# chellmuth/pathed

Hardware: AMD Instinct MI355X
Metric: Msamples/s (pixels x spp / s), PathTracer radiance loop (higher is better)
Workload: dtype f32; 1 GPU; scenes/cornell.json 1024x1024, 1024 spp per step x 8 steps = 8192 spp, bounces 0..10, seed 1; total_samples=8589934592, parallelism=the samples of every step split over 1 GPU(s), no exchange

## Files before the change

### include/pathed_hip.h

```cpp
#ifndef PATHED_HIP_H
#define PATHED_HIP_H

#include <stddef.h>
#include <stdint.h>

#ifdef __cplusplus
extern "C" {
#endif

#define PATHED_ABI_VERSION 4

#define PATHED_OK            0
#define PATHED_E_INVALID    -1
#define PATHED_E_DEVICE     -2
#define PATHED_E_NO_DEVICE  -3
#define PATHED_E_UNSUPPORTED -4
#define PATHED_E_NOMEM      -5

#define PATHED_MAT_LAMBERTIAN 0
#define PATHED_MAT_OREN_NAYAR 1
#define PATHED_MAT_MICROFACET 2
#define PATHED_MAT_PLASTIC    3
#define PATHED_MAT_GLASS      4
#define PATHED_MAT_MIRROR     5
// ... 270 lines not shown
};
enum {
    PATHED_TRAITS_ALL = 0, PATHED_TRAITS_LAMBERTIAN_TRIANGLES = 1, PATHED_TRAITS_LAMBERTIAN_PLASTIC_SPHERES = 2,
    PATHED_TRAITS_LAMBERTIAN_GLASS_CONTAINER = 3, PATHED_TRAITS_TRIANGLE_LIT = 4, PATHED_TRAITS_ENVIRONMENT_ONLY = 5,
    PATHED_TRAITS_ROUGH_BECKMANN = 6, PATHED_TRAITS_ROUGH_GGX = 7, PATHED_TRAITS_SMOOTH = 8, PATHED_TRAITS_COUNT = 9
};
int pathed_hip_debug_shading_queries(PathedScene *scene, int function, int traits, size_t n, const float *in, float *out);

int pathed_hip_debug_phase_samples(PathedScene *scene, size_t n, const float *u, float *out);

int pathed_hip_trace(PathedScene *scene, const float *rays, size_t n,
                     int any_hit, void *hits);

int pathed_hip_debug_small_candidates(PathedScene *scene, const float *rays, size_t n, uint64_t *out);

int pathed_hip_debug_camera_masks(PathedScene *scene, uint64_t *out, size_t n_pixels);

int pathed_hip_debug_item_order(PathedScene *scene, int32_t *primitives, size_t n_triangles);

int pathed_hip_debug_light_records(PathedScene *scene, float *triangles, size_t n_triangles, float *lights, size_t max_lights, int *n_lights);

int pathed_hip_debug_instance_records(PathedScene *scene, float *records , size_t n_instances);

int pathed_hip_has_experiments(void);

int pathed_hip_set_stats_mode(PathedScene *scene, int enabled);
int pathed_hip_get_stats(PathedScene *scene, PathedStats *out);
int pathed_hip_reset_stats(PathedScene *scene);

int pathed_hip_scene_export_bvh(PathedScene *scene,
// ... 40 lines not shown
```

### pathed_amd/_capi.py

```python
import ctypes as C
import os

_HERE = os.path.dirname(os.path.abspath(__file__))
REPO_ROOT = os.path.dirname(_HERE)
LIB_DIR = os.path.join(_HERE, "lib")

PATHED_ABI_VERSION = 4

MAT_LAMBERTIAN, MAT_OREN_NAYAR, MAT_MICROFACET, MAT_PLASTIC, MAT_GLASS, MAT_MIRROR, MAT_PASSTHROUGH = range(7)
INTEGRATOR_PATH_TRACER, INTEGRATOR_VOLUME_PATH_TRACER, INTEGRATOR_ALBEDO, INTEGRATOR_BASIC_VOLUME = 0, 1, 2, 3
ALBEDO_CONSTANT, ALBEDO_CHECKERBOARD, ALBEDO_TEXTURE = 0, 1, 2
GEOM_MESH, GEOM_SPHERE = 0, 1


class PathedCamera(C.Structure):
    _fields_ = [
        ("origin", C.c_float * 3),
        ("target", C.c_float * 3),
        ("up", C.c_float * 3),
        ("vertical_fov", C.c_float),
        ("width", C.c_int32),
        ("height", C.c_int32),
        ("flip_handedness", C.c_int32),
    ]
# ... 211 lines not shown
    "pathed_hip_grid_queries",
    "pathed_hip_debug_shading_queries",
    "pathed_hip_debug_phase_samples",
    "pathed_hip_scene_destroy",
    "pathed_hip_render",
    "pathed_hip_render_device",
    "pathed_hip_render_features",
    "pathed_hip_render_features_device",
    "pathed_hip_render_moments",
    "pathed_hip_render_moments_device",
    "pathed_hip_noise_estimate_device",
    "pathed_hip_select_pixels_device",
    "pathed_hip_render_pixels_device",
    "pathed_hip_trace",
    "pathed_hip_debug_small_candidates",
    "pathed_hip_debug_camera_masks",
    "pathed_hip_debug_item_order",
    "pathed_hip_debug_light_records",
    "pathed_hip_has_experiments",
    "pathed_hip_scene_refit",
    "pathed_hip_set_samples_per_unit",
    "pathed_hip_set_integrator",
    "pathed_hip_set_stats_mode",
    "pathed_hip_get_stats",
    "pathed_hip_reset_stats",
    "pathed_hip_scene_export_bvh",
    "pathed_hip_scene_export_compressed_nodes",
    "pathed_hip_measure_bandwidth",
    "pathed_hip_measure_valu",
    "pathed_hip_measure_valu_modes",
# ... 102 lines not shown
        lib.pathed_hip_render_moments_device.argtypes = [vp, C.c_uint64, C.c_uint32, C.c_uint32, C.c_int, C.c_int, vp, vp, vp]
        lib.pathed_hip_render_moments_device.restype = C.c_int
        lib.pathed_hip_render_moments.argtypes = [vp, C.c_uint64, C.c_uint32, C.c_uint32, C.c_int, C.c_int, fp, fp]
        lib.pathed_hip_render_moments.restype = C.c_int
        lib.pathed_hip_noise_estimate_device.argtypes = [vp, vp, vp, C.c_uint32, C.c_float, C.c_float, vp, C.POINTER(PathedNoise), vp]
        lib.pathed_hip_noise_estimate_device.restype = C.c_int
    if hasattr(lib, "pathed_hip_render_pixels_device"):
        lib.pathed_hip_select_pixels_device.argtypes = [vp, vp, vp, vp, C.c_float, C.c_float, vp, vp, C.POINTER(C.c_uint32), C.POINTER(PathedNoise), vp]
        lib.pathed_hip_select_pixels_device.restype = C.c_int
        lib.pathed_hip_render_pixels_device.argtypes = [vp, C.c_uint64, C.c_uint32, C.c_uint32, C.c_int, C.c_int, vp, C.c_uint32, vp, vp, vp, vp]
        lib.pathed_hip_render_pixels_device.restype = C.c_int
    lib.pathed_hip_trace.argtypes = [vp, C.POINTER(C.c_float), C.c_size_t, C.c_int, vp]
    lib.pathed_hip_trace.restype = C.c_int
    lib.pathed_hip_debug_small_candidates.argtypes = [vp, C.POINTER(C.c_float), C.c_size_t, C.POINTER(C.c_uint64)]
    lib.pathed_hip_debug_small_candidates.restype = C.c_int
    lib.pathed_hip_debug_light_records.argtypes = [vp, C.POINTER(C.c_float), C.c_size_t, C.POINTER(C.c_float), C.c_size_t, C.POINTER(C.c_int)]
    lib.pathed_hip_debug_light_records.restype = C.c_int
    if hasattr(lib, "pathed_hip_debug_camera_masks"):
        lib.pathed_hip_debug_camera_masks.argtypes = [vp, C.POINTER(C.c_uint64), C.c_size_t]
        lib.pathed_hip_debug_camera_masks.restype = C.c_int
        lib.pathed_hip_debug_item_order.argtypes = [vp, C.POINTER(C.c_int32), C.c_size_t]
        lib.pathed_hip_debug_item_order.restype = C.c_int
    if hasattr(lib, "pathed_hip_debug_shading_queries"):
        lib.pathed_hip_debug_shading_queries.argtypes = [vp, C.c_int, C.c_int, C.c_size_t, C.POINTER(C.c_float), C.POINTER(C.c_float)]
        lib.pathed_hip_debug_shading_queries.restype = C.c_int
    if hasattr(lib, "pathed_hip_debug_phase_samples"):
        lib.pathed_hip_debug_phase_samples.argtypes = [vp, C.c_size_t, C.POINTER(C.c_float), C.POINTER(C.c_float)]
        lib.pathed_hip_debug_phase_samples.restype = C.c_int
    lib.pathed_hip_scene_refit.argtypes = [vp, C.POINTER(C.c_float), C.POINTER(C.c_float), C.c_uint32, C.POINTER(C.c_float)]
    lib.pathed_hip_scene_refit.restype = C.c_int
# ... 79 lines not shown
```

### pathed_amd/csrc/kernels.h

```cpp
#pragma once

#ifndef PATHED_RESOLVE_SHARED
#define PATHED_RESOLVE_SHARED 2
#endif
#ifndef PATHED_EXPERIMENTS
#define PATHED_EXPERIMENTS 0
#endif
#include "mfma_candidates.h"
#include "small_items.h"
#include "camera_masks.h"
#include "shading.h"
#include "trace.h"
#include "volume.h"

namespace pathed {

static const int kBlock = 256;
static_assert(kBlock == kVolumeBlock, "volume.h indexes the LDS stack rows with the block size");
static const int kWavesPerBlock = kBlock / 64;
static const int kMaxLdsMaterials = 96;
#ifndef PATHED_UNIT_QUEUES
#define PATHED_UNIT_QUEUES 32
#endif
static const int kUnitQueues = PATHED_UNIT_QUEUES;
// ... 733 lines not shown
    } else {
        aHigh = 0u;
        bHigh = 0u;
    }
    *lowA = aLow; *highA = aHigh; *lowB = bLow; *highB = bHigh;
}

__device__ __forceinline__ unsigned int shiftInBit(unsigned int word, unsigned long long laneMask)
{
    unsigned int result;
    unsigned long long carryOut;
    asm("v_addc_co_u32_e64 %0, %1, %2, %2, %3" : "=v"(result), "=s"(carryOut) : "v"(word), "s"(laneMask));
    return result;
}

template <bool SHADOW, bool QUADS = true, bool LONE = true>
__device__ __forceinline__ void smallCandidatesItems(const f2 *records, int nQuads, int nTris, float kappaT, V3 origin, V3 directionA, V3 directionB,
                                                     unsigned int *lowA, unsigned int *highA, unsigned int *lowB, unsigned int *highB,
                                                     float tnearLow, float tfarHighB)
{
    unsigned int loA = 0u, hiA = 0u, loB = 0u, hiB = 0u;
    const f2 ax = splat2(directionA.x), ay = splat2(directionA.y), az = splat2(directionA.z);
    const f2 bx = splat2(directionB.x), by = splat2(directionB.y), bz = splat2(directionB.z);
    const f2 ox = splat2(origin.x), oy = splat2(origin.y), oz = splat2(origin.z);
    const f2 nearLow = splat2(-tnearLow), farHighB = splat2(fminf(tfarHighB, 1e30f));
    const f2 kappaLength = splat2(kappaT);

    const int nQuadPairs = QUADS ? (nQuads + 1) >> 1 : 0;
    for (int pair = 0; QUADS && pair < nQuadPairs; pair++) {
        const f2 *record = records + kSmallQuadWords * pair;
        const f2 c0x = record[0], c0y = record[1], c0z = record[2];
        const f2 a1x = record[3], a1y = record[4], a1z = record[5];
        const f2 a2x = record[6], a2y = record[7], a2z = record[8];
        const f2 k2UV = record[9], amaxSquared = record[10], k2T = record[11], cD = record[13], kappaUV = record[15];
        const f2 tx = ox - c0x, ty = oy - c0y, tz = oz - c0z;
        const f2 qx = fma2(ty, a1z, -(tz * a1y));
        const f2 qy = fma2(tz, a1x, -(tx * a1z));
        const f2 qz = fma2(tx, a1y, -(ty * a1x));
        const f2 tScaled = fma2(a2x, qx, fma2(a2y, qy, a2z * qz));
        const f2 tt = fma2(tx, tx, fma2(ty, ty, tz * tz));
        const f2 reachSquared = tt + amaxSquared;
        const f2 originUV = k2UV * reachSquared, originT = k2T * reachSquared;
        auto oneRay = [&](f2 dx, f2 dy, f2 dz, bool far, unsigned int &lo, unsigned int &hi) {
            const f2 px = fma2(dy, a2z, -(dz * a2y));
// ... 17 lines not shown
                const f2 farBound = fma2(farHighB, det, -tScaled) * det;
                const f2 tolFar = fma2(farHighB, fma2(splat2(kSmallKappaFar), dd, cD), tolT);
                rejectX |= PATHED_LANES(farBound.x < -tolFar.x);
                rejectY |= PATHED_LANES(farBound.y < -tolFar.y);
            }
            const f2 twice = tolUV + tolUV;
            const float twiceX = twice.x, twiceY = twice.y;
            hi = __builtin_amdgcn_alignbit(hi, lo, 28);
            lo = shiftInBit(lo, ~(rejectX | PATHED_LANES(diagonal.x < -twiceX)));
            lo = shiftInBit(lo, ~(rejectX | PATHED_LANES(diagonal.x > twiceX)));
            lo = shiftInBit(lo, ~(rejectY | PATHED_LANES(diagonal.y < -twiceY)));
            lo = shiftInBit(lo, ~(rejectY | PATHED_LANES(diagonal.y > twiceY)));
        };
        oneRay(ax, ay, az, false, loA, hiA);
        __builtin_amdgcn_sched_barrier(0);
        if (SHADOW) { oneRay(bx, by, bz, true, loB, hiB); }
        __builtin_amdgcn_sched_barrier(0);
    }
    unsigned long long accA, accB;
    if (QUADS && (nQuads & 1)) {
        accA = (((unsigned long long)hiA << 32) | loA) >> 2; accB = (((unsigned long long)hiB << 32) | loB) >> 2;
        loA = (unsigned int)accA; hiA = (unsigned int)(accA >> 32); loB = (unsigned int)accB; hiB = (unsigned int)(accB >> 32);
    }

    const f2 *lone = records + kSmallQuadWords * nQuadPairs;
    const int nLone = LONE ? nTris - 2 * nQuads : 0;
    const int nLonePairs = (nLone + 1) >> 1;
    for (int pair = 0; LONE && pair < nLonePairs; pair++) {
        const f2 *record = lone + kSmallPairWords * pair;
        const f2 v0x = record[0], v0y = record[1], v0z = record[2];
        const f2 e1x = record[3], e1y = record[4], e1z = record[5];
        const f2 e2x = record[6], e2y = record[7], e2z = record[8];
        const f2 tx = ox - v0x, ty = oy - v0y, tz = oz - v0z;
        const f2 qx = fma2(ty, e1z, -(tz * e1y));
// ... 9 lines not shown
            const f2 vScaled = fma2(dx, qx, fma2(dy, qy, dz * qz));
            const f2 a = uScaled * det, b = vScaled * det, c = (det - (uScaled + vScaled)) * det, e = fma2(nearLow, det, tScaled) * det;
            float worstA = fminf(fminf(a.x, b.x), fminf(c.x, e.x));
            float worstB = fminf(fminf(a.y, b.y), fminf(c.y, e.y));
            if (far) {
                const f2 g = fma2(splat2(tfarHighB), det, -tScaled) * det;
                worstA = fminf(worstA, g.x);
                worstB = fminf(worstB, g.y);
            }
            hi = __builtin_amdgcn_alignbit(hi, lo, 30);
            lo = shiftInBit(lo, ~PATHED_LANES(worstA < 0.f));
            lo = shiftInBit(lo, ~PATHED_LANES(worstB < 0.f));
            #undef PATHED_LANES
        };
        oneRay(ax, ay, az, false, loA, hiA);
        if (SHADOW) { oneRay(bx, by, bz, true, loB, hiB); }
    }
    accA = ((unsigned long long)hiA << 32) | loA; accB = ((unsigned long long)hiB << 32) | loB;
    if (LONE && (nLone & 1)) { accA >>= 1; accB >>= 1; }

    const int shift = 64 - nTris;
    accA <<= shift;
    accB <<= shift;
    *lowA = (unsigned int)(accA >> 32); *highA = (unsigned int)accA; *lowB = (unsigned int)(accB >> 32); *highB = (unsigned int)accB;
}

__device__ __forceinline__ void smallResolve(const TraceGeometry &geometry, LaneRay &ray, unsigned int candidatesLow, unsigned int candidatesHigh)
{
    while (__ballot((candidatesLow | candidatesHigh) != 0u) != 0ull) {
        if ((candidatesLow | candidatesHigh) != 0u) {
            int k;
            if (candidatesLow != 0u) { k = __clz((int)candidatesLow); candidatesLow &= ~(0x80000000u >> k); }
            else { k = __clz((int)candidatesHigh); candidatesHigh &= ~(0x80000000u >> k); k += 32; }
            const float4 t0 = geometry.tris[3 * k + 0];
            const float4 t1 = geometry.tris[3 * k + 1];
            const float4 t2 = geometry.tris[3 * k + 2];
            bool terminate = false;
            testLeafTriangle(ray, t0, t1, t2, &terminate);
            if (terminate) { candidatesLow = 0u; candidatesHigh = 0u; }
        }
// ... 1974 lines not shown
        LaneRay ray;
        laneRayInit(ray, path.o, path.d, PATHED_TNEAR, PATHED_TFAR, false);
        {
            const bool traceShadow = tracing && pendingShadow;
            LaneRay shadowRay;
            laneRayInit(shadowRay, path.o, shadowDirection, PATHED_TNEAR, shadowTfar, true);
            unsigned int candidatesLow = 0, candidatesHigh = 0, shadowLow = 0, shadowHigh = 0;
            SHADE_REGION(2, traceShadow);
            if (MFMA) {
                mfmaCandidatesPair(mfmaRows, nTris, p.mfmaFrame, __ballot(traceShadow) != 0ull, path.o, path.d, shadowDirection,
                                   candidateNear(PATHED_TNEAR), candidateFar(shadowTfar), &candidatesLow, &candidatesHigh, &shadowLow, &shadowHigh);
                if (!tracing) { candidatesLow = 0u; candidatesHigh = 0u; }
                if (!traceShadow) { shadowLow = 0u; shadowHigh = 0u; }
            } else if (QUADS) {
                if (tracing) {
                    smallCandidatesItems<true, true, true>(smallTris.data, p.smallQuads, nTris, p.smallKappaT, path.o, path.d, shadowDirection,
                                                            &candidatesLow, &candidatesHigh, &shadowLow, &shadowHigh,
                                                            candidateNear(PATHED_TNEAR), candidateFar(shadowTfar));
                    if (!traceShadow) { shadowLow = 0u; shadowHigh = 0u; }
                }
            } else if (__ballot(traceShadow) != 0ull) {
                if (tracing) {
                    smallCandidatesPair(smallTris.data, nTris, path.o, path.d, shadowDirection, &candidatesLow, &candidatesHigh, &shadowLow, &shadowHigh,
                                        candidateNear(PATHED_TNEAR), candidateFar(shadowTfar));
                    if (!traceShadow) { shadowLow = 0u; shadowHigh = 0u; }
                }
            } else if (tracing) {
                smallCandidates(smallTris.data, nTris, path.o, path.d, &candidatesLow, &candidatesHigh, candidateNear(PATHED_TNEAR));
            }
            if (COUNT && tracing) {
                trisTested += (unsigned int)nTris * (traceShadow ? 2u : 1u);
                closestRays++;
                if (traceShadow) { shadowRays++; }
// ... 158 lines not shown
        if (((k < 32 ? aLow : aHigh) >> (31 - (k & 31))) & 1u) { valuA |= bit; }
        if (((k < 32 ? bLow : bHigh) >> (31 - (k & 31))) & 1u) { valuB |= bit; }
        if ((((k & 1) ? oddA : evenA) >> (k >> 1)) & 1u) { mfmaA |= bit; }
        if ((((k & 1) ? oddB : evenB) >> (k >> 1)) & 1u) { mfmaB |= bit; }
        float t, u, v;
        if (intersectTriangle(o, dA, v3(t0.x, t0.y, t0.z), v3(t1.x, t1.y, t1.z), v3(t2.x, t2.y, t2.z), &t, &u, &v) && t > PATHED_TNEAR && t <= PATHED_TFAR) { acceptA |= bit; }
        if (intersectTriangle(o, dB, v3(t0.x, t0.y, t0.z), v3(t1.x, t1.y, t1.z), v3(t2.x, t2.y, t2.z), &t, &u, &v) && t > PATHED_TNEAR && t <= tfarB) { acceptB |= bit; }
        const unsigned long long itemBit = 1ull << (floatAsInt(itemTris[3 * k].w) & 63);
        if (((k < 32 ? iaLow : iaHigh) >> (31 - (k & 31))) & 1u) { itemsA |= itemBit; }
        if (((k < 32 ? ibLow : ibHigh) >> (31 - (k & 31))) & 1u) { itemsB |= itemBit; }
    }
    if (index < n) {
        unsigned long long *row = out + (size_t)8 * index;
        row[0] = valuA; row[1] = valuB; row[2] = mfmaA; row[3] = mfmaB; row[4] = acceptA; row[5] = acceptB; row[6] = itemsA; row[7] = itemsB;
    }
}

template <bool QUADS = false, typename MaterialTable>
__device__ __forceinline__ bool volumeQuerySmall(const VolumeContext<MaterialTable> &c, const f2 *pairRecords, int smallQuads, float smallKappaT,
                                                 int mode, V3 o, V3 d, float tfar, RayHit *hit, VolumeEvents *eventsOut)
{
    LaneRay ray;
    const bool anyHit = mode == kQueryVolumeOccluded;
    laneRayInit(ray, o, d, PATHED_TNEAR, tfar, anyHit);
    VolumeEvents events;
    eventsClear(events);
    unsigned int low = 0u, high = 0u;
    if (QUADS) {
        unsigned int unusedLow = 0u, unusedHigh = 0u;
        smallCandidatesItems<true>(pairRecords, smallQuads, c.geometry.nTris, smallKappaT, o, d, d, &unusedLow, &unusedHigh, &low, &high,
// ... 915 lines not shown
```

### pathed_amd/csrc/pathed_hip.hip

```cpp
#include "pathed_hip.h"

#include "bvh_build.h"
#include "kernels.h"
#include "features.h"
#include "shading_queries.h"
#if PATHED_EXPERIMENTS
#include "kernels_experiments.h"
#endif
#include "lbvh.h"

#include <hip/hip_runtime.h>

#include <dlfcn.h>

#include <chrono>
#include <cmath>
#include <cstdio>
#include <cstdlib>
#include <cstring>
#include <mutex>
#include <string>
#include <type_traits>
#include <vector>

// ... 223 lines not shown
    unsigned int listCap = 0;
    DeviceBuffer<unsigned int> slotLists, deferredLists;
    size_t deferredSlots = 0;
    int stageRounds = 2;

    int stackRows = 8;
    int maxStack = 0;
    bool sceneInLds = false;
    bool bruteForce = false;
    SmallTris smallTris;
    SmallTris smallItems;
    SmallItemsLayout smallLayout;
    DeviceBuffer<float4> itemTris;
    std::vector<float> itemTrisHost;
    std::vector<float> smallExtraPoints;
    bool refittable = false;
    DeviceBuffer<float> soupPositions, soupNormals, soupUvs;
    DeviceBuffer<uint32_t> soupIndices;
    DeviceBuffer<int> soupTriMaterial;
    DeviceBuffer<float4> refitLo, refitHi;
    DeviceBuffer<unsigned char> refitReady;
    size_t soupVertices = 0;
    int localCount = 0;
    float4 localTris[3 * 8];
    float localLo[3] = { 0.f, 0.f, 0.f }, localHi[3] = { 0.f, 0.f, 0.f }, localSphere[4] = { 0.f, 0.f, 0.f, 0.f };
    bool hybridAvailable = false;
    bool hybridPath = false;
    SmallTris hybridItems;
    SmallItemsLayout hybridLayout;
    std::vector<float> hybridDirectLeaf;
// ... 879 lines not shown
        if (!strcmp(text, "tiles")) { return kOrderTiles; }
        if (!strcmp(text, "stripes-tiled")) { return kOrderStripesTiled; }
        if (!strcmp(text, "stripes")) { return kOrderStripes; }
    }
    return fallback;
}

static hipError_t rebuildSmallItems(PathedScene *scene)
{
    if (!scene->bruteForce || scene->device.nTris <= 0) { return hipSuccess; }
    std::vector<float> points = scene->smallExtraPoints;
    for (int a = 0; a < 3; a++) { points.push_back(scene->device.camera.origin[a]); }
    const int kMaxQuadMaterials = 64;
    const bool pairQuads = scene->options.generic_kernels == 0 && !tuningEnv("PATHED_NO_QUADS") && scene->device.nMaterials <= kMaxQuadMaterials;
    std::vector<float> ordered;
    scene->smallLayout = buildSmallItems(scene->bvh.leafTris.data(), scene->device.nTris, points.data(), (int)(points.size() / 3), pairQuads, PATHED_TNEAR,
                                         reinterpret_cast<float *>(scene->smallItems.data), &ordered);
    std::vector<float4> records(ordered.size() / 4);
    std::memcpy(records.data(), ordered.data(), ordered.size() * sizeof(float));
    scene->itemTrisHost = ordered;
    const hipError_t status = scene->itemTris.upload(records);
    if (status == hipSuccess && scene->mfmaPhase1) {
        std::vector<float> table;
        buildMfmaTable(scene->itemTrisHost.data(), scene->device.nTris, scene->device.camera.origin, 1, &table, &scene->mfmaFrame);
        return scene->mfmaTable.upload(table);
    }
    return status;
}

static size_t cameraQueueWords(const PathedScene *scene)
{
    const size_t queueBlocks = (size_t)(scene->computeUnits > 0 ? scene->computeUnits : 1) * PATHED_FUSED_WAVES;
// ... 911 lines not shown
        for (int k = 0; k < scene->device.nTris; k++) {
            const float *tri = tris + (size_t)12 * k;
            f2 *record = scene->smallTris.data + (size_t)kSmallPairWords * (k / 2);
            for (int row = 0; row < 3; row++) {
                for (int axis = 0; axis < 3; axis++) { record[3 * row + axis][k & 1] = tri[4 * row + axis]; }
            }
        }
    }
    std::memset(&scene->smallItems, 0, sizeof scene->smallItems);
    scene->smallExtraPoints.clear();
    for (uint32_t i = 0; i < desc->n_spheres; i++) {
        for (int sign = -1; sign <= 1; sign += 2) {
            for (int a = 0; a < 3; a++) { scene->smallExtraPoints.push_back(desc->spheres[i].center_world[a] + sign * std::fabs(desc->spheres[i].radius) * 1.001f); }
        }
    }
    if ((status = rebuildSmallItems(scene)) != hipSuccess) { return fail_cleanup(status, "upload the phase-1 records"); }
    scene->mfmaPhase1 = false;
    std::memset(&scene->mfmaFrame, 0, sizeof scene->mfmaFrame);
    if (scene->bruteForce && scene->fusedPath) {
        int phase1 = options.small_phase1;
        if (const char *text = tuningEnv("PATHED_SMALL_PHASE1")) {
            if (!strcmp(text, "valu")) { phase1 = 1; } else if (!strcmp(text, "mfma")) { phase1 = 2; }
        }
        if (phase1 == 0) { phase1 = kDefaultSmallPhase1; }
        if (phase1 == 2 && scene->device.nTris > 0) {
            std::vector<float> table;
            buildMfmaTable(scene->itemTrisHost.data(), scene->device.nTris, scene->device.camera.origin, 1, &table, &scene->mfmaFrame);
            if ((status = scene->mfmaTable.upload(table)) != hipSuccess) { return fail_cleanup(status, "upload the matrix-pipe rows"); }
            scene->mfmaPhase1 = true;
        }
// ... 220 lines not shown
        std::memcpy(params.spherePairs, scene->spherePairs, sizeof params.spherePairs);

        const SceneTraitFlags &traits = scene->traits;
        const bool count = scene->countMode;
        const auto run = [&](void (*kernel)(RenderParams, SmallTris)) { hipLaunchKernelGGL(kernel, grid, dim3(kBlock), lds, stream, params, scene->smallItems); };
#if PATHED_EXPERIMENTS
        if (scene->mfmaPhase1 && ldsMaterials) {
            withBool(count, [&](auto COUNT) {
                if (traits.lambertianTriangles) { run(k_path_small<true, COUNT, TraitsLambertianTriangles, true>); }
                else if (traits.lambertianPlasticSpheres) { run(k_path_small<true, COUNT, TraitsLambertianPlasticSpheres, true>); }
                else { run(k_path_small<true, COUNT, TraitsAll, true>); }
            });
        } else
#endif
        if (scene->smallLayout.nQuads > 0 && ldsMaterials) {
            if (traits.lambertianTriangles) { withBool(count, [&](auto COUNT) { run(k_path_small<true, COUNT, TraitsLambertianTriangles, false, true>); }); }
            else if (traits.lambertianPlasticSpheres) { withBool(count, [&](auto COUNT) { run(k_path_small<true, COUNT, TraitsLambertianPlasticSpheres, false, true>); }); }
            else if (traits.roughBeckmann && !count) { run(k_path_small<true, false, TraitsRoughBeckmann, false, true>); }
            else if (traits.roughGgx && !count) { run(k_path_small<true, false, TraitsRoughGgx, false, true>); }
            else if (traits.smoothSet && !count) { run(k_path_small<true, false, TraitsSmooth, false, true>); }
            else if (traits.triangleLit && !count) { run(k_path_small<true, false, TraitsTriangleLit, false, true>); }
            else { withBool(count, [&](auto COUNT) { run(k_path_small<true, COUNT, TraitsAll, false, true>); }); }
        } else if (traits.lambertianTriangles) {
            withBool(ldsMaterials, [&](auto LDS_MATERIALS) { withBool(count, [&](auto COUNT) { run(k_path_small<LDS_MATERIALS, COUNT, TraitsLambertianTriangles>); }); });
        } else if (traits.lambertianPlasticSpheres && ldsMaterials) {
            withBool(count, [&](auto COUNT) { run(k_path_small<true, COUNT, TraitsLambertianPlasticSpheres>); });
        } else {
            withBool(ldsMaterials, [&](auto LDS_MATERIALS) { withBool(count, [&](auto COUNT) { run(k_path_small<LDS_MATERIALS, COUNT, TraitsAll>); }); });
        }
    });
    if (queueShort) { return fail(PATHED_E_DEVICE, "the fused kernel's grid outgrew its camera queues"); }
    return code;
}

static int renderPassVolume(PathedScene *scene, const Pass &pass)
{
    if (pass.nList > 0) {
// ... 1054 lines not shown
    std::memcpy(hostRays.data(), rays, n * 10 * sizeof(float));
    for (size_t i = n; i < padded; i++) { hostRays[10 * i + 5] = 1.f; hostRays[10 * i + 8] = 1.f; }
    DeviceBuffer<float> deviceRays;
    DeviceBuffer<unsigned long long> deviceOut;
    HIP_TRY(deviceRays.upload(hostRays));
    HIP_TRY(deviceOut.allocate(n * 8));
    hipLaunchKernelGGL(k_debug_small_candidates, dim3((unsigned)(padded / kBlock)), dim3(kBlock), 0, nullptr, scene->device, scene->smallTris,
                       scene->smallItems, scene->smallLayout.nQuads, scene->smallLayout.kappaT, scene->itemTris.ptr, table.ptr, frame,
                       deviceRays.ptr, (int)n, deviceOut.ptr);
    HIP_TRY(hipGetLastError());
    HIP_TRY(hipDeviceSynchronize());
    HIP_TRY(hipMemcpy(out, deviceOut.ptr, n * 8 * sizeof(unsigned long long), hipMemcpyDeviceToHost));
    return PATHED_OK;
}

int pathed_hip_debug_camera_masks(PathedScene *scene, uint64_t *out, size_t n_pixels)
{
    if (!scene || !out) { return fail(PATHED_E_INVALID, "null scene or output buffer"); }
    if (!scene->bruteForce || !scene->fusedPath) { return fail(PATHED_E_UNSUPPORTED, "only scenes on the fused path kernel carry camera-ray candidate masks"); }
    if (n_pixels != (size_t)scene->width * (size_t)scene->height) { return fail(PATHED_E_INVALID, "n_pixels must be the scene's pixel count"); }
    SELECT_DEVICE(scene);
    if (!scene->cameraMasksBuilt) { HIP_TRY(rebuildCameraMasks(scene)); }
    HIP_TRY(hipMemcpy(out, scene->cameraQueue.ptr, n_pixels * sizeof(uint64_t), hipMemcpyDeviceToHost));
    return PATHED_OK;
}

int pathed_hip_debug_item_order(PathedScene *scene, int32_t *primitives, size_t n_triangles)
{
    if (!scene || !primitives) { return fail(PATHED_E_INVALID, "null scene or output buffer"); }
    if (!scene->bruteForce) { return fail(PATHED_E_UNSUPPORTED, "the all-triangles intersector serves scenes of 1..64 triangles"); }
// ... 402 lines not shown
```

### pathed_amd/csrc/small_items.h

```cpp
#pragma once

#include <algorithm>
#include <cmath>
#include <cstring>
#include <vector>

namespace pathed {

static const int kSmallQuadWords = 16;
static const int kSmallLoneWords = 9;
static const int kSmallItemFloats = 2 * 9 * 32;
static const float kSmallKappa = 1e-5f;
static const float kSmallKappaFar = 1e-6f;

struct SmallItemsLayout {
    int nQuads = 0;
    int nLone = 0;
    float kappaT = 0.f;
};

inline SmallItemsLayout buildSmallItems(const float *leafTris, int nTris, const float *extraPoints, int nExtra, bool pairQuads, float tnear,
                                        float *records, std::vector<float> *itemTris)
{
    SmallItemsLayout layout;
    std::memset(records, 0, sizeof(float) * kSmallItemFloats);
    itemTris->assign((size_t)12 * std::max(nTris, 1), 0.f);
    struct Corners { double p[3][3]; };
    std::vector<Corners> corners((size_t)nTris);
    double lo[3] = { 1e300, 1e300, 1e300 }, hi[3] = { -1e300, -1e300, -1e300 };
    auto cover = [&](const double *point) {
        for (int a = 0; a < 3; a++) { lo[a] = std::min(lo[a], point[a]); hi[a] = std::max(hi[a], point[a]); }
    };
    for (int k = 0; k < nTris; k++) {
        const float *tri = leafTris + (size_t)12 * k;
        for (int a = 0; a < 3; a++) {
            corners[k].p[0][a] = tri[a];
            corners[k].p[1][a] = (double)tri[a] + (double)tri[4 + a];
// ... 91 lines not shown
            quads.push_back(quad);
            break;
        }
    }
    auto floatsNeeded = [&](size_t nQuads) {
        return (size_t)2 * kSmallQuadWords * ((nQuads + 1) / 2) + (size_t)2 * kSmallLoneWords * (((size_t)nTris - 2 * nQuads + 1) / 2);
    };
    while (!quads.empty() && floatsNeeded(quads.size()) > (size_t)kSmallItemFloats) {
        partner[quads.back().a] = -1;
        partner[quads.back().b] = -1;
        quads.pop_back();
    }
    layout.nQuads = (int)quads.size();
    layout.nLone = nTris - 2 * layout.nQuads;

    const double kappa = kSmallKappa, kappaT = layout.kappaT;
    for (int q = 0; q < layout.nQuads; q++) {
        const Quad &quad = quads[q];
        float *record = records + (size_t)2 * kSmallQuadWords * (q / 2);
        const int half = q & 1;
        const double zero[3] = { 0.0, 0.0, 0.0 };
        const double amax = quad.amax;
        const double eUV = 1.01 * (32.0 * unit * amax + 4.0 * quad.delta);
        const double area = distance(quad.a1, zero) * distance(quad.a2, zero);
        const double eT = 1.01 * (32.0 * unit * area + 8.0 * quad.delta * amax);
        const double eDet = 1.01 * (16.0 * unit * area + 4.0 * quad.delta * amax);
        const double k2UV = 1.5 * (eUV * eUV / (2.0 * kappa) + eDet / 2.0);
        const double k2T = 1.5 * (eT * eT / (2.0 * std::max(kappaT, 1e-300)) + eDet * area / (2.0 * std::max(amax, 1e-300)));
        const double cD = 1.5 * eDet * eDet / (4.0 * kSmallKappaFar);
        for (int x = 0; x < 3; x++) {
            record[2 * (0 + x) + half] = (float)quad.c0[x];
            record[2 * (3 + x) + half] = (float)quad.a1[x];
            record[2 * (6 + x) + half] = (float)quad.a2[x];
        }
        record[2 * 9 + half] = (float)std::max(k2UV, 1e-37);
        record[2 * 10 + half] = (float)std::max(amax * amax * 1.000001, 1e-37);
        record[2 * 11 + half] = (float)std::max(k2T, 1e-37);
        record[2 * 13 + half] = (float)std::max(cD, 1e-37);
        record[2 * 14 + half] = (float)std::max(eDet, 1e-37);
        record[2 * 15 + half] = (float)(kappa + 1.0001 * quad.excess);
        std::memcpy(itemTris->data() + (size_t)12 * (2 * q), leafTris + (size_t)12 * quad.a, 12 * sizeof(float));
        std::memcpy(itemTris->data() + (size_t)12 * (2 * q + 1), leafTris + (size_t)12 * quad.b, 12 * sizeof(float));
    }
    float *lone = records + (size_t)2 * kSmallQuadWords * ((layout.nQuads + 1) / 2);
    int k = 0;
    for (int t = 0; t < nTris; t++) {
        if (partner[t] >= 0) { continue; }
        const float *tri = leafTris + (size_t)12 * t;
        float *record = lone + (size_t)2 * kSmallLoneWords * (k / 2);
        for (int row = 0; row < 3; row++) {
            for (int axis = 0; axis < 3; axis++) { record[2 * (3 * row + axis) + (k & 1)] = tri[4 * row + axis]; }
        }
        std::memcpy(itemTris->data() + (size_t)12 * (2 * layout.nQuads + k), tri, 12 * sizeof(float));
        k++;
    }
    return layout;
}

}
```

### pathed_amd/integrator.py

```python
import ctypes as C

import numpy as np

from . import _capi


class PathedError(RuntimeError):
    pass


def _check(lib, code, what):
    if code != 0:
        raise PathedError("%s failed (%d): %s" % (what, code, lib.pathed_hip_last_error().decode()))


SEED_RANGE = "an integer in [0, 2^64)"


def _seed(seed):
    if isinstance(seed, bool) or not isinstance(seed, (int, np.integer)) or not 0 <= int(seed) < 1 << 64:
        raise PathedError("seed must be %s, not %r" % (SEED_RANGE, seed))
    return int(seed)


# ... 283 lines not shown
        out = np.zeros(n, dtype=np.int32) if any_hit else np.zeros((n, 4), dtype=np.float32)
        code = self._lib.pathed_hip_trace(
            self._handle, rays.ctypes.data_as(C.POINTER(C.c_float)), n, 1 if any_hit else 0,
            out.ctypes.data_as(C.c_void_p))
        _check(self._lib, code, "pathed_hip_trace")
        return out

    def small_candidates(self, rays):
        rays = np.ascontiguousarray(rays, dtype=np.float32).reshape(-1, 10)
        out = np.zeros((rays.shape[0], 8), dtype=np.uint64)
        code = self._lib.pathed_hip_debug_small_candidates(
            self._handle, rays.ctypes.data_as(C.POINTER(C.c_float)), rays.shape[0], out.ctypes.data_as(C.POINTER(C.c_uint64)))
        _check(self._lib, code, "pathed_hip_debug_small_candidates")
        return out

    def camera_masks(self):
        out = np.zeros((self.height, self.width), dtype=np.uint64)
        code = self._lib.pathed_hip_debug_camera_masks(self._handle, out.ctypes.data_as(C.POINTER(C.c_uint64)), out.size)
        _check(self._lib, code, "pathed_hip_debug_camera_masks")
        return out

    def item_order(self, n_triangles):
        out = np.zeros(n_triangles, dtype=np.int32)
        code = self._lib.pathed_hip_debug_item_order(self._handle, out.ctypes.data_as(C.POINTER(C.c_int32)), n_triangles)
        _check(self._lib, code, "pathed_hip_debug_item_order")
        return out

    def light_records(self, n_triangles, max_lights):
        triangles = np.zeros((n_triangles, 20), dtype=np.float32)
        lights = np.zeros((max_lights, 18), dtype=np.float32)
# ... 332 lines not shown
```

Measured before the change: 3308 Msamples/s.

## Skip shadow tests against triangles proven never to occlude light paths

Adds a host-side geometric proof that marks triangles which can never occlude a shadow ray toward an emitter (all other geometry lies on one side of their plane, with emitters far enough away). Quads and lone triangles are reordered so the possible occluders come first, and the Lambertian-triangle small-scene kernel tests shadow rays only against that prefix, shifting the masks to keep bit positions. This cuts per-bounce shadow candidate work in Cornell-like scenes whose walls cannot shadow the light, at the cost of extra packing into the smallQuads parameter and a conservative error-bound analysis that must hold for correctness.

```diff
diff --git a/include/pathed_hip.h b/include/pathed_hip.h
--- a/include/pathed_hip.h
+++ b/include/pathed_hip.h
@@ -308,6 +308,8 @@
 
 int pathed_hip_debug_small_candidates(PathedScene *scene, const float *rays, size_t n, uint64_t *out);
 
+int pathed_hip_debug_shadow_candidates(PathedScene *scene, const float *rays, size_t n, uint64_t *out, int32_t *layout, uint64_t *never_occluders);
+
 int pathed_hip_debug_camera_masks(PathedScene *scene, uint64_t *out, size_t n_pixels);
 
 int pathed_hip_debug_item_order(PathedScene *scene, int32_t *primitives, size_t n_triangles);
diff --git a/pathed_amd/_capi.py b/pathed_amd/_capi.py
--- a/pathed_amd/_capi.py
+++ b/pathed_amd/_capi.py
@@ -249,6 +249,7 @@
     "pathed_hip_render_pixels_device",
     "pathed_hip_trace",
     "pathed_hip_debug_small_candidates",
+    "pathed_hip_debug_shadow_candidates",
     "pathed_hip_debug_camera_masks",
     "pathed_hip_debug_item_order",
     "pathed_hip_debug_light_records",
@@ -381,6 +382,8 @@
     lib.pathed_hip_trace.restype = C.c_int
     lib.pathed_hip_debug_small_candidates.argtypes = [vp, C.POINTER(C.c_float), C.c_size_t, C.POINTER(C.c_uint64)]
     lib.pathed_hip_debug_small_candidates.restype = C.c_int
+    lib.pathed_hip_debug_shadow_candidates.argtypes = [vp, C.POINTER(C.c_float), C.c_size_t, C.POINTER(C.c_uint64), C.POINTER(C.c_int32), C.POINTER(C.c_uint64)]
+    lib.pathed_hip_debug_shadow_candidates.restype = C.c_int
     lib.pathed_hip_debug_light_records.argtypes = [vp, C.POINTER(C.c_float), C.c_size_t, C.POINTER(C.c_float), C.c_size_t, C.POINTER(C.c_int)]
     lib.pathed_hip_debug_light_records.restype = C.c_int
     if hasattr(lib, "pathed_hip_debug_camera_masks"):
diff --git a/pathed_amd/csrc/kernels.h b/pathed_amd/csrc/kernels.h
--- a/pathed_amd/csrc/kernels.h
+++ b/pathed_amd/csrc/kernels.h
@@ -771,10 +771,10 @@
     return result;
 }
 
-template <bool SHADOW, bool QUADS = true, bool LONE = true>
+template <bool SHADOW, bool QUADS = true, bool LONE = true, bool PRUNE = false>
 __device__ __forceinline__ void smallCandidatesItems(const f2 *records, int nQuads, int nTris, float kappaT, V3 origin, V3 directionA, V3 directionB,
                                                      unsigned int *lowA, unsigned int *highA, unsigned int *lowB, unsigned int *highB,
-                                                     float tnearLow, float tfarHighB)
+                                                     float tnearLow, float tfarHighB, int shadowQuadPairs = 0, int shadowLonePairs = 0)
 {
     unsigned int loA = 0u, hiA = 0u, loB = 0u, hiB = 0u;
     const f2 ax = splat2(directionA.x), ay = splat2(directionA.y), az = splat2(directionA.z);
@@ -784,7 +784,7 @@
     const f2 kappaLength = splat2(kappaT);
 
     const int nQuadPairs = QUADS ? (nQuads + 1) >> 1 : 0;
-    for (int pair = 0; QUADS && pair < nQuadPairs; pair++) {
+    auto quadTurn = [&](int pair, bool withShadow) __attribute__((always_inline)) {
         const f2 *record = records + kSmallQuadWords * pair;
         const f2 c0x = record[0], c0y = record[1], c0z = record[2];
         const f2 a1x = record[3], a1y = record[4], a1z = record[5];
@@ -832,10 +832,17 @@
         };
         oneRay(ax, ay, az, false, loA, hiA);
         __builtin_amdgcn_sched_barrier(0);
-        if (SHADOW) { oneRay(bx, by, bz, true, loB, hiB); }
+        if (withShadow) { oneRay(bx, by, bz, true, loB, hiB); }
         __builtin_amdgcn_sched_barrier(0);
-    }
+    };
+    const int bothPairs = PRUNE ? (shadowQuadPairs < nQuadPairs ? shadowQuadPairs : nQuadPairs) : nQuadPairs;
+    for (int pair = 0; QUADS && pair < bothPairs; pair++) { quadTurn(pair, SHADOW); }
+    for (int pair = bothPairs; PRUNE && QUADS && pair < nQuadPairs; pair++) { quadTurn(pair, false); }
     unsigned long long accA, accB;
+    if (PRUNE && QUADS && SHADOW) {
+        accB = (((unsigned long long)hiB << 32) | loB) << ((4 * (nQuadPairs - bothPairs)) & 63);
+        loB = (unsigned int)accB; hiB = (unsigned int)(accB >> 32);
+    }
     if (QUADS && (nQuads & 1)) {
         accA = (((unsigned long long)hiA << 32) | loA) >> 2; accB = (((unsigned long long)hiB << 32) | loB) >> 2;
         loA = (unsigned int)accA; hiA = (unsigned int)(accA >> 32); loB = (unsigned int)accB; hiB = (unsigned int)(accB >> 32);
@@ -875,9 +882,10 @@
             #undef PATHED_LANES
         };
         oneRay(ax, ay, az, false, loA, hiA);
-        if (SHADOW) { oneRay(bx, by, bz, true, loB, hiB); }
+        if (SHADOW && (!PRUNE || pair < shadowLonePairs)) { oneRay(bx, by, bz, true, loB, hiB); }
     }
     accA = ((unsigned long long)hiA << 32) | loA; accB = ((unsigned long long)hiB << 32) | loB;
+    if (PRUNE && LONE && SHADOW) { accB <<= (2 * (nLonePairs - shadowLonePairs)) & 63; }
     if (LONE && (nLone & 1)) { accA >>= 1; accB >>= 1; }
 
     const int shift = 64 - nTris;
@@ -885,6 +893,10 @@
     accB <<= shift;
     *lowA = (unsigned int)(accA >> 32); *highA = (unsigned int)accA; *lowB = (unsigned int)(accB >> 32); *highB = (unsigned int)accB;
 }
+
+template <bool COUNT, typename TRAITS>
+constexpr bool kSmallPrunes = !COUNT && std::is_same<TRAITS, TraitsLambertianTriangles>::value;
+template <typename TRAITS> struct TraitsTag { typedef TRAITS type; };
 
 __device__ __forceinline__ void smallResolve(const TraceGeometry &geometry, LaneRay &ray, unsigned int candidatesLow, unsigned int candidatesHigh)
 {
@@ -2889,9 +2901,12 @@
                 if (!traceShadow) { shadowLow = 0u; shadowHigh = 0u; }
             } else if (QUADS) {
                 if (tracing) {
-                    smallCandidatesItems<true, true, true>(smallTris.data, p.smallQuads, nTris, p.smallKappaT, path.o, path.d, shadowDirection,
-                                                            &candidatesLow, &candidatesHigh, &shadowLow, &shadowHigh,
-                                                            candidateNear(PATHED_TNEAR), candidateFar(shadowTfar));
+                    constexpr bool kPrune = kSmallPrunes<COUNT, TRAITS>;
+                    const int smallQuads = kPrune ? (p.smallQuads & 0xFFFF) : p.smallQuads;
+                    smallCandidatesItems<true, true, true, kPrune>(smallTris.data, smallQuads, nTris, p.smallKappaT, path.o, path.d, shadowDirection,
+                                                                   &candidatesLow, &candidatesHigh, &shadowLow, &shadowHigh,
+                                                                   candidateNear(PATHED_TNEAR), candidateFar(shadowTfar),
+                                                                   (p.smallQuads >> 16) & 0xFF, (p.smallQuads >> 24) & 0xFF);
                     if (!traceShadow) { shadowLow = 0u; shadowHigh = 0u; }
                 }
             } else if (__ballot(traceShadow) != 0ull) {
@@ -3080,6 +3095,28 @@
         unsigned long long *row = out + (size_t)8 * index;
         row[0] = valuA; row[1] = valuB; row[2] = mfmaA; row[3] = mfmaB; row[4] = acceptA; row[5] = acceptB; row[6] = itemsA; row[7] = itemsB;
     }
+}
+
+__global__ __launch_bounds__(kBlock) void k_debug_shadow_candidates(DScene scene, SmallTris smallItems, int nQuads, float kappaT, int shadowQuadPairs, int shadowLonePairs,
+                                                                    const float4 *itemTris, const float *rays, int n, unsigned long long *out)
+{
+    const int index = blockIdx.x * kBlock + threadIdx.x;
+    const float *r = rays + (size_t)10 * index;
+    const V3 o = v3(r[0], r[1], r[2]), dA = v3(r[3], r[4], r[5]), dB = v3(r[6], r[7], r[8]);
+    const float tfarB = r[9];
+    const int nTris = scene.nTris;
+    unsigned int aLow, aHigh, bLow, bHigh;
+    smallCandidatesItems<true, true, true, true>(smallItems.data, nQuads, nTris, kappaT, o, dA, dB, &aLow, &aHigh, &bLow, &bHigh,
+                                                 candidateNear(PATHED_TNEAR), candidateFar(tfarB), shadowQuadPairs, shadowLonePairs);
+    unsigned long long candidates = 0, accepted = 0;
+    for (int k = 0; k < nTris; k++) {
+        const float4 t0 = itemTris[3 * k + 0], t1 = itemTris[3 * k + 1], t2 = itemTris[3 * k + 2];
+        const unsigned long long bit = 1ull << (floatAsInt(t0.w) & 63);
+        if (((k < 32 ? bLow : bHigh) >> (31 - (k & 31))) & 1u) { candidates |= bit; }
+        float t, u, v;
+        if (intersectTriangle(o, dB, v3(t0.x, t0.y, t0.z), v3(t1.x, t1.y, t1.z), v3(t2.x, t2.y, t2.z), &t, &u, &v) && t > PATHED_TNEAR && t <= tfarB) { accepted |= bit; }
+    }
+    if (index < n) { out[(size_t)2 * index] = candidates; out[(size_t)2 * index + 1] = accepted; }
 }
 
 template <bool QUADS = false, typename MaterialTable>
diff --git a/pathed_amd/csrc/pathed_hip.hip b/pathed_amd/csrc/pathed_hip.hip
--- a/pathed_amd/csrc/pathed_hip.hip
+++ b/pathed_amd/csrc/pathed_hip.hip
@@ -261,6 +261,8 @@
     DeviceBuffer<float4> itemTris;
     std::vector<float> itemTrisHost;
     std::vector<float> smallExtraPoints;
+    std::vector<unsigned char> smallEmitterPrims;
+    std::vector<float> smallSphereLights;
     bool refittable = false;
     DeviceBuffer<float> soupPositions, soupNormals, soupUvs;
     DeviceBuffer<uint32_t> soupIndices;
@@ -1170,8 +1172,23 @@
     const int kMaxQuadMaterials = 64;
     const bool pairQuads = scene->options.generic_kernels == 0 && !tuningEnv("PATHED_NO_QUADS") && scene->device.nMaterials <= kMaxQuadMaterials;
     std::vector<float> ordered;
+    std::vector<unsigned char> emitter((size_t)scene->device.nTris, 0);
+    bool lightsKnown = true;
+    for (int k = 0; k < scene->device.nTris; k++) {
+        int prim;
+        std::memcpy(&prim, &scene->bvh.leafTris[(size_t)12 * k + 3], sizeof prim);
+        if (prim < 0 || (size_t)prim >= scene->smallEmitterPrims.size()) { lightsKnown = false; break; }
+        emitter[(size_t)k] = scene->smallEmitterPrims[(size_t)prim];
+    }
+    SmallLights lights;
+    lights.known = lightsKnown;
+    lights.environment = scene->device.hasEnv != 0;
+    lights.emitter = emitter.data();
+    lights.spheres = scene->smallSphereLights.data();
+    lights.nSpheres = (int)(scene->smallSphereLights.size() / 4);
+    lights.nSurfacePoints = (int)(scene->smallExtraPoints.size() / 3);
     scene->smallLayout = buildSmallItems(scene->bvh.leafTris.data(), scene->device.nTris, points.data(), (int)(points.size() / 3), pairQuads, PATHED_TNEAR,
-                                         reinterpret_cast<float *>(scene->smallItems.data), &ordered);
+                                         reinterpret_cast<float *>(scene->smallItems.data), &ordered, &lights);
     std::vector<float4> records(ordered.size() / 4);
     std::memcpy(records.data(), ordered.data(), ordered.size() * sizeof(float));
     scene->itemTrisHost = ordered;
@@ -2113,6 +2130,17 @@
             for (int a = 0; a < 3; a++) { scene->smallExtraPoints.push_back(desc->spheres[i].center_world[a] + sign * std::fabs(desc->spheres[i].radius) * 1.001f); }
         }
     }
+    scene->smallEmitterPrims.assign((size_t)desc->n_triangles, 0);
+    scene->smallSphereLights.clear();
+    for (const DLight &light : lights) {
+        if (light.kind == 0 && light.index >= 0 && (size_t)light.index < scene->smallEmitterPrims.size()) { scene->smallEmitterPrims[(size_t)light.index] = 1; }
+        if (light.kind == 1) {
+            for (int a = 0; a < 3; a++) { scene->smallSphereLights.push_back(desc->spheres[light.index].center_sample[a]); }
+            scene->smallSphereLights.push_back(desc->spheres[light.index].radius);
+            for (int a = 0; a < 3; a++) { scene->smallSphereLights.push_back(desc->spheres[light.index].center_world[a]); }
+            scene->smallSphereLights.push_back(desc->spheres[light.index].radius);
+        }
+    }
     if ((status = rebuildSmallItems(scene)) != hipSuccess) { return fail_cleanup(status, "upload the phase-1 records"); }
     scene->mfmaPhase1 = false;
     std::memset(&scene->mfmaFrame, 0, sizeof scene->mfmaFrame);
@@ -2363,13 +2391,21 @@
         } else
 #endif
         if (scene->smallLayout.nQuads > 0 && ldsMaterials) {
-            if (traits.lambertianTriangles) { withBool(count, [&](auto COUNT) { run(k_path_small<true, COUNT, TraitsLambertianTriangles, false, true>); }); }
-            else if (traits.lambertianPlasticSpheres) { withBool(count, [&](auto COUNT) { run(k_path_small<true, COUNT, TraitsLambertianPlasticSpheres, false, true>); }); }
-            else if (traits.roughBeckmann && !count) { run(k_path_small<true, false, TraitsRoughBeckmann, false, true>); }
-            else if (traits.roughGgx && !count) { run(k_path_small<true, false, TraitsRoughGgx, false, true>); }
-            else if (traits.smoothSet && !count) { run(k_path_small<true, false, TraitsSmooth, false, true>); }
-            else if (traits.triangleLit && !count) { run(k_path_small<true, false, TraitsTriangleLit, false, true>); }
-            else { withBool(count, [&](auto COUNT) { run(k_path_small<true, COUNT, TraitsAll, false, true>); }); }
+            const auto quadsKernel = [&](auto COUNT, auto traitsTag) -> void (*)(RenderParams, SmallTris) {
+                using TRAITS = typename decltype(traitsTag)::type;
+                if (kSmallPrunes<decltype(COUNT)::value, TRAITS>) {
+                    params.smallQuads = scene->smallLayout.nQuads | scene->smallLayout.shadowQuadPairs << 16 | scene->smallLayout.shadowLonePairs << 24;
+                }
+                return k_path_small<true, decltype(COUNT)::value, TRAITS, false, true>;
+            };
+            const std::false_type plain{};
+            if (traits.lambertianTriangles) { withBool(count, [&](auto COUNT) { run(quadsKernel(COUNT, TraitsTag<TraitsLambertianTriangles>())); }); }
+            else if (traits.lambertianPlasticSpheres) { withBool(count, [&](auto COUNT) { run(quadsKernel(COUNT, TraitsTag<TraitsLambertianPlasticSpheres>())); }); }
+            else if (traits.roughBeckmann && !count) { run(quadsKernel(plain, TraitsTag<TraitsRoughBeckmann>())); }
+            else if (traits.roughGgx && !count) { run(quadsKernel(plain, TraitsTag<TraitsRoughGgx>())); }
+            else if (traits.smoothSet && !count) { run(quadsKernel(plain, TraitsTag<TraitsSmooth>())); }
+            else if (traits.triangleLit && !count) { run(quadsKernel(plain, TraitsTag<TraitsTriangleLit>())); }
+            else { withBool(count, [&](auto COUNT) { run(quadsKernel(COUNT, TraitsTag<TraitsAll>())); }); }
         } else if (traits.lambertianTriangles) {
             withBool(ldsMaterials, [&](auto LDS_MATERIALS) { withBool(count, [&](auto COUNT) { run(k_path_small<LDS_MATERIALS, COUNT, TraitsLambertianTriangles>); }); });
         } else if (traits.lambertianPlasticSpheres && ldsMaterials) {
@@ -3454,6 +3490,38 @@
     return PATHED_OK;
 }
 
+int pathed_hip_debug_shadow_candidates(PathedScene *scene, const float *rays, size_t n, uint64_t *out, int32_t *layout, uint64_t *never_occluders)
+{
+    if (!scene) { return fail(PATHED_E_INVALID, "null scene"); }
+    if (scene->instanced) { return fail(PATHED_E_UNSUPPORTED, "the all-triangles intersector's hook does not serve scenes with instances"); }
+    if (!scene->bruteForce || scene->device.nTris < 1) { return fail(PATHED_E_UNSUPPORTED, "the all-triangles intersector serves scenes of 1..64 triangles"); }
+    if (!layout || !never_occluders) { return fail(PATHED_E_INVALID, "null layout or never-occluder buffer"); }
+    layout[0] = scene->smallLayout.nQuads;
+    layout[1] = scene->smallLayout.nLone;
+    layout[2] = scene->smallLayout.shadowQuadPairs;
+    layout[3] = scene->smallLayout.shadowLonePairs;
+    *never_occluders = scene->smallLayout.neverOccluders;
+    if (n == 0) { return PATHED_OK; }
+    if (!rays || !out) { return fail(PATHED_E_INVALID, "null ray or output buffer"); }
+    if (n > (size_t)1 << 24) { return fail(PATHED_E_INVALID, "too many rays in one call"); }
+    SELECT_DEVICE(scene);
+    const size_t padded = (n + kBlock - 1) / kBlock * kBlock;
+    std::vector<float> hostRays(padded * 10, 0.f);
+    std::memcpy(hostRays.data(), rays, n * 10 * sizeof(float));
+    for (size_t i = n; i < padded; i++) { hostRays[10 * i + 5] = 1.f; hostRays[10 * i + 8] = 1.f; }
+    DeviceBuffer<float> deviceRays;
+    DeviceBuffer<unsigned long long> deviceOut;
+    HIP_TRY(deviceRays.upload(hostRays));
+    HIP_TRY(deviceOut.allocate(n * 2));
+    hipLaunchKernelGGL(k_debug_shadow_candidates, dim3((unsigned)(padded / kBlock)), dim3(kBlock), 0, nullptr, scene->device, scene->smallItems,
+                       scene->smallLayout.nQuads, scene->smallLayout.kappaT, scene->smallLayout.shadowQuadPairs, scene->smallLayout.shadowLonePairs,
+                       scene->itemTris.ptr, deviceRays.ptr, (int)n, deviceOut.ptr);
+    HIP_TRY(hipGetLastError());
+    HIP_TRY(hipDeviceSynchronize());
+    HIP_TRY(hipMemcpy(out, deviceOut.ptr, n * 2 * sizeof(unsigned long long), hipMemcpyDeviceToHost));
+    return PATHED_OK;
+}
+
 int pathed_hip_debug_camera_masks(PathedScene *scene, uint64_t *out, size_t n_pixels)
 {
     if (!scene || !out) { return fail(PATHED_E_INVALID, "null scene or output buffer"); }
diff --git a/pathed_amd/csrc/small_items.h b/pathed_amd/csrc/small_items.h
--- a/pathed_amd/csrc/small_items.h
+++ b/pathed_amd/csrc/small_items.h
@@ -17,10 +17,123 @@
     int nQuads = 0;
     int nLone = 0;
     float kappaT = 0.f;
+    int shadowQuadPairs = 0;
+    int shadowLonePairs = 0;
+    unsigned long long neverOccluders = 0ull;
+    double eta = 0.0, dMin = 0.0;
 };
 
+struct SmallLights {
+    bool known = false;
+    bool environment = false;
+    const unsigned char *emitter = nullptr;
+    const float *spheres = nullptr;
+    int nSpheres = 0;
+    int nSurfacePoints = 0;
+};
+
+inline void smallNeverOccluders(const float *leafTris, int nTris, const float *extraPoints, int nExtra, const SmallLights &lights, float tnear,
+                                std::vector<unsigned char> *marks, double *etaOut = nullptr, double *dMinOut = nullptr)
+{
+    marks->assign((size_t)std::max(nTris, 0), 0);
+    if (etaOut) { *etaOut = 0.0; }
+    if (dMinOut) { *dMinOut = 0.0; }
+    if (!lights.known || lights.environment || nTris <= 0 || !lights.emitter || !(tnear > 0.f)) { return; }
+    const double unit = 1.0 / 16777216.0;
+    const int nSurface = std::min(std::max(lights.nSurfacePoints, 0), nExtra) & ~1;
+    struct Tri { double p[3][3], k; };
+    std::vector<Tri> tris((size_t)nTris);
+    double lo[3] = { 1e300, 1e300, 1e300 }, hi[3] = { -1e300, -1e300, -1e300 }, sLo[3], sHi[3], largest = 0.0, kMax = 0.0;
+    auto cover = [&](const double *point) {
+        for (int a = 0; a < 3; a++) { lo[a] = std::min(lo[a], point[a]); hi[a] = std::max(hi[a], point[a]); largest = std::max(largest, std::fabs(point[a])); }
+    };
+    auto cross = [](const double *a, const double *b, double *out) {
+        out[0] = a[1] * b[2] - a[2] * b[1]; out[1] = a[2] * b[0] - a[0] * b[2]; out[2] = a[0] * b[1] - a[1] * b[0];
+    };
+    auto norm = [](const double *a) { return std::sqrt(a[0] * a[0] + a[1] * a[1] + a[2] * a[2]); };
+    for (int t = 0; t < nTris; t++) {
+        const float *tri = leafTris + (size_t)12 * t;
+        double e1[3], e2[3], n[3];
+        for (int a = 0; a < 3; a++) {
+            e1[a] = tri[4 + a]; e2[a] = tri[8 + a];
+            tris[t].p[0][a] = tri[a]; tris[t].p[1][a] = (double)tri[a] + e1[a]; tris[t].p[2][a] = (double)tri[a] + e2[a];
+        }
+        for (int c = 0; c < 3; c++) { cover(tris[t].p[c]); }
+        cross(e1, e2, n);
+        const double area2 = norm(n), edges = norm(e1) * norm(e2);
+        tris[t].k = area2 > 0.0 ? edges / area2 : 1e300;
+        if (!(tris[t].k >= 1.0)) { tris[t].k = 1e300; }
+        if (!(edges == 0.0)) { kMax = std::max(kMax, tris[t].k); }
+    }
+    for (int i = 0; i < nSurface; i++) {
+        const double point[3] = { extraPoints[3 * i], extraPoints[3 * i + 1], extraPoints[3 * i + 2] };
+        cover(point);
+    }
+    for (int a = 0; a < 3; a++) { sLo[a] = lo[a]; sHi[a] = hi[a]; }
+    for (int i = nSurface; i < nExtra; i++) {
+        const double point[3] = { extraPoints[3 * i], extraPoints[3 * i + 1], extraPoints[3 * i + 2] };
+        cover(point);
+    }
+    auto diagonal = [](const double *from, const double *to) {
+        double sum = 0.0;
+        for (int a = 0; a < 3; a++) { if (to[a] > from[a]) { sum += (to[a] - from[a]) * (to[a] - from[a]); } }
+        return std::sqrt(sum) * 1.001;
+    };
+    const double R = diagonal(lo, hi), L = diagonal(sLo, sHi);
+    const double eta = 1.01 * (unit * R + 16.0 * unit * R * kMax) + 1.01 * 3.0 * unit * (largest + R);
+    const double etaSphere = 1.1 * std::sqrt(32.0 * unit) * R;
+    const double dMin = eta + 2.0 * eta * L * 4.0 / tnear;
+    const double emitterSlack = 16.0 * unit * largest;
+    if (!(eta > 0.0) || !(dMin > 0.0) || !(dMin < 1e300)) { return; }
+    if (etaOut) { *etaOut = eta; }
+    if (dMinOut) { *dMinOut = dMin; }
+    bool anyEmitter = lights.nSpheres > 0;
+    for (int t = 0; t < nTris; t++) { anyEmitter = anyEmitter || lights.emitter[t] != 0; }
+    if (!anyEmitter) { return; }
+
+    for (int y = 0; y < nTris; y++) {
+        const Tri &Y = tris[y];
+        const double climb = dMin / (2.0 * L) - 8.0 * unit * Y.k;
+        if (!(climb > 0.0)) { continue; }
+        const double eT = 1.01 * 8.0 * unit * (L + tnear) * Y.k / climb + unit * tnear;
+        if (!(eT <= 0.5 * tnear)) { continue; }
+        if (!(0.5 * dMin > 1.01 * 16.0 * unit * L * Y.k)) { continue; }
+        double e1[3], e2[3], n[3];
+        for (int a = 0; a < 3; a++) { e1[a] = Y.p[1][a] - Y.p[0][a]; e2[a] = Y.p[2][a] - Y.p[0][a]; }
+        cross(e1, e2, n);
+        const double length = norm(n);
+        if (!(length > 1e-12 * norm(e1) * norm(e2)) || !(length > 0.0)) { continue; }
+        for (int a = 0; a < 3; a++) { n[a] /= length; }
+        for (int orientation = 0; orientation < 2 && !(*marks)[y]; orientation++) {
+            const double sign = orientation ? -1.0 : 1.0;
+            const double c = sign * (n[0] * Y.p[0][0] + n[1] * Y.p[0][1] + n[2] * Y.p[0][2]);
+            auto s = [&](const double *x) { return sign * (n[0] * x[0] + n[1] * x[1] + n[2] * x[2]) - c; };
+            bool holds = true;
+            for (int corner = 0; corner < 3 && holds; corner++) { holds = std::fabs(s(Y.p[corner])) <= eta; }
+            for (int t = 0; t < nTris && holds; t++) {
+                for (int corner = 0; corner < 3 && holds; corner++) {
+                    const double value = s(tris[t].p[corner]);
+                    holds = value >= -eta && (!lights.emitter[t] || value >= dMin + emitterSlack);
+                }
+            }
+            for (int i = 0; i + 1 < nSurface && holds; i += 2) {
+                const float *a = extraPoints + 3 * i, *b = a + 3;
+                double least = -c;
+                for (int x = 0; x < 3; x++) { least += std::min(sign * n[x] * (double)a[x], sign * n[x] * (double)b[x]); }
+                holds = least >= etaSphere;
+            }
+            for (int i = 0; i < lights.nSpheres && holds; i++) {
+                const float *sphere = lights.spheres + 4 * i;
+                const double centre[3] = { sphere[0], sphere[1], sphere[2] };
+                holds = s(centre) - std::fabs((double)sphere[3]) * 1.001 >= dMin + emitterSlack;
+            }
+            if (holds) { (*marks)[y] = 1; }
+        }
+    }
+}
+
 inline SmallItemsLayout buildSmallItems(const float *leafTris, int nTris, const float *extraPoints, int nExtra, bool pairQuads, float tnear,
-                                        float *records, std::vector<float> *itemTris)
+                                        float *records, std::vector<float> *itemTris, const SmallLights *lights = nullptr)
 {
     SmallItemsLayout layout;
     std::memset(records, 0, sizeof(float) * kSmallItemFloats);
@@ -142,6 +255,25 @@
     layout.nQuads = (int)quads.size();
     layout.nLone = nTris - 2 * layout.nQuads;
 
+    std::vector<unsigned char> never;
+    smallNeverOccluders(leafTris, nTris, extraPoints, nExtra, lights ? *lights : SmallLights(), tnear, &never, &layout.eta, &layout.dMin);
+    auto neverQuad = [&](const Quad &quad) { return never[quad.a] && never[quad.b]; };
+    std::stable_partition(quads.begin(), quads.end(), [&](const Quad &quad) { return !neverQuad(quad); });
+    int occluderQuads = 0, occluderLone = 0;
+    for (const Quad &quad : quads) { occluderQuads += neverQuad(quad) ? 0 : 1; }
+    std::vector<int> loneOrder;
+    for (int pass = 0; pass < 2; pass++) {
+        for (int t = 0; t < nTris; t++) {
+            if (partner[t] < 0 && (never[t] != 0) == (pass == 1)) { loneOrder.push_back(t); }
+        }
+        if (pass == 0) { occluderLone = (int)loneOrder.size(); }
+    }
+    layout.shadowQuadPairs = (occluderQuads + 1) / 2;
+    layout.shadowLonePairs = (occluderLone + 1) / 2;
+    auto primitive = [&](int t) { int id; std::memcpy(&id, leafTris + (size_t)12 * t + 3, sizeof id); return id; };
+    for (int q = occluderQuads; q < layout.nQuads; q++) { layout.neverOccluders |= 1ull << (primitive(quads[q].a) & 63) | 1ull << (primitive(quads[q].b) & 63); }
+    for (int k = occluderLone; k < layout.nLone; k++) { layout.neverOccluders |= 1ull << (primitive(loneOrder[k]) & 63); }
+
     const double kappa = kSmallKappa, kappaT = layout.kappaT;
     for (int q = 0; q < layout.nQuads; q++) {
         const Quad &quad = quads[q];
@@ -172,8 +304,7 @@
     }
     float *lone = records + (size_t)2 * kSmallQuadWords * ((layout.nQuads + 1) / 2);
     int k = 0;
-    for (int t = 0; t < nTris; t++) {
-        if (partner[t] >= 0) { continue; }
+    for (int t : loneOrder) {
         const float *tri = leafTris + (size_t)12 * t;
         float *record = lone + (size_t)2 * kSmallLoneWords * (k / 2);
         for (int row = 0; row < 3; row++) {
diff --git a/pathed_amd/integrator.py b/pathed_amd/integrator.py
--- a/pathed_amd/integrator.py
+++ b/pathed_amd/integrator.py
@@ -321,6 +321,17 @@
         _check(self._lib, code, "pathed_hip_debug_small_candidates")
         return out
 
+    def shadow_candidates(self, rays):
+        rays = np.ascontiguousarray(rays, dtype=np.float32).reshape(-1, 10)
+        out = np.zeros((rays.shape[0], 2), dtype=np.uint64)
+        layout = (C.c_int32 * 4)()
+        never = C.c_uint64(0)
+        code = self._lib.pathed_hip_debug_shadow_candidates(
+            self._handle, rays.ctypes.data_as(C.POINTER(C.c_float)), rays.shape[0], out.ctypes.data_as(C.POINTER(C.c_uint64)), layout, C.byref(never))
+        _check(self._lib, code, "pathed_hip_debug_shadow_candidates")
+        counts = {"quads": layout[0], "lone": layout[1], "shadow_quad_pairs": layout[2], "shadow_lone_pairs": layout[3]}
+        return out, counts, int(never.value)
+
     def camera_masks(self):
         out = np.zeros((self.height, self.width), dtype=np.uint64)
         code = self._lib.pathed_hip_debug_camera_masks(self._handle, out.ctypes.data_as(C.POINTER(C.c_uint64)), out.size)
```

Measured after the change: 3472 Msamples/s, median of 6. +5.0%, better.
